# yhw-yhw/TalkSHOW

Hardware: NVIDIA H100
Metric: smplx_motion_frames_per_sec (higher is better)
Workload: dtype f32

## Files before the change

talkshow_b200/csrc/face.cu:

```cuda
#include <cuda_fp16.h>
#include "convstack.h"

#include <memory>
#include "pixelcnn.h"

namespace ts {

static const int W2V_K[7] = {10, 3, 3, 3, 3, 2, 2};
static const int W2V_S[7] = {5, 2, 2, 2, 2, 2, 2};

struct EncLayer {
  Layer qkv, out, ff1, ff2;
  float *ln1_g, *ln1_b, *ln2_g, *ln2_b;
};

struct FaceNet {
  float* conv0_w = nullptr;
  float *gn_g = nullptr, *gn_b = nullptr;
  Layer conv[7];
  float *fp_ln_g = nullptr, *fp_ln_b = nullptr;
  Layer fproj, posconv;
  unsigned short* pos_w16 = nullptr;
  float pos_unscale = 1.f;
  float *enc_ln_g = nullptr, *enc_ln_b = nullptr;
  std::vector<EncLayer> layers;
  Layer feat_map;
  float *id_w = nullptr, *id_b = nullptr;
  int ncls = 4;
  Layer fn_conv[3], fn_res0;
  float *fn_g[3], *fn_b[3];
  Layer dec_conv[2][3];
  float *dec_g[2][3], *dec_b[2][3];
  Layer fin[2];
  int jaw_dim = 3, exp_dim = 100;
};

void face_destroy(ts_engine* e) {
  delete e->face;
  e->face = nullptr;
}

static float* up(ts_engine* e, const float* p, size_t n) { return e->upload(std::vector<float>(p, p + n)); }

static Layer pack_ckc(ts_engine* e, const float* w, const float* b, int cout, int cin, int k) {
  int cp = pad4(cin);
  std::vector<float> W((size_t)cout * k * cp, 0.f);
  for (int o = 0; o < cout; ++o)
    for (int c = 0; c < cin; ++c)
      for (int t = 0; t < k; ++t) W[((size_t)o * k + t) * cp + c] = w[((size_t)o * cin + c) * k + t];
  Layer L;
  L.N = cout; L.taps = k; L.cin = cp; L.K = k * cp;
  upload_weights(e, W, &L);
  L.bias = b ? up(e, b, cout) : nullptr;
  return L;
}
static Layer pack_linear(ts_engine* e, const float* w, const float* b, int N, int K) {
  Layer L;
  L.N = N; L.K = K; L.taps = 1; L.cin = K;
  upload_weights(e, std::vector<float>(w, w + (size_t)N * K), &L);
  L.bias = b ? up(e, b, N) : nullptr;
  return L;
}

__global__ void __launch_bounds__(256) conv0_stats_kernel(const float* __restrict__ wave, const float* __restrict__ w, int N, int T0,
                                                          double* __restrict__ stats) {
  constexpr int TC = 256;
  __shared__ float xs[TC * 5 + 16];
  const int b = blockIdx.y, t0 = blockIdx.x * TC, tid = threadIdx.x;
  const int nt = min(TC, T0 - t0);
  const float* x = wave + (size_t)b * N + (size_t)t0 * 5;
  for (int i = tid; i < nt * 5 + 5; i += 256) xs[i] = x[i];
  __syncthreads();
  for (int c = tid; c < 512; c += 256) {
    float wr[10];
#pragma unroll
    for (int j = 0; j < 10; ++j) wr[j] = w[c * 10 + j];
    double s = 0.0, ss = 0.0;
    for (int t = 0; t < nt; ++t) {
      float y = 0.f;
#pragma unroll
      for (int j = 0; j < 10; ++j) y = fmaf(wr[j], xs[t * 5 + j], y);
      s += (double)y;
      ss += (double)y * (double)y;
    }
    atomicAdd(&stats[((size_t)b * 512 + c) * 2], s);
    atomicAdd(&stats[((size_t)b * 512 + c) * 2 + 1], ss);
  }
}
__global__ void __launch_bounds__(256) conv0_apply_kernel(const float* __restrict__ wave, const float* __restrict__ w,
                                                          const double* __restrict__ stats, const float* __restrict__ g,
                                                          const float* __restrict__ bta, int N, int T0, Act3 out) {
  constexpr int TC = 64;
  __shared__ float xs[TC * 5 + 16];
  const int b = blockIdx.y, t0 = blockIdx.x * TC, tid = threadIdx.x;
  const int nt = min(TC, T0 - t0);
  const float* x = wave + (size_t)b * N + (size_t)t0 * 5;
  for (int i = tid; i < nt * 5 + 5; i += 256) xs[i] = x[i];
  __syncthreads();
  for (int c = tid; c < 512; c += 256) {
    float wr[10];
#pragma unroll
    for (int j = 0; j < 10; ++j) wr[j] = w[c * 10 + j];
    double s = stats[((size_t)b * 512 + c) * 2], ss = stats[((size_t)b * 512 + c) * 2 + 1];
    double mean = s / T0, var = ss / T0 - mean * mean;
    if (var < 0) var = 0;
    float rstd = (float)(1.0 / sqrt(var + 1e-5)), mu = (float)mean, gg = g[c], bb = bta[c];
    for (int t = 0; t < nt; ++t) {
      float y = 0.f;
#pragma unroll
      for (int j = 0; j < 10; ++j) y = fmaf(wr[j], xs[t * 5 + j], y);
      float v = (y - mu) * rstd * gg + bb;
      v = 0.5f * v * (1.0f + erff(v * 0.70710678118654752440f));
      if (out.h16) {
        if (out.p) out.row(b, t0 + t)[c] = v;
        split16(v, out.row_h16(b, t0 + t)[c], out.row_l16(b, t0 + t)[c]);
      } else if (out.lo) {
        float h = __uint_as_float(__float_as_uint(v) & 0xffffe000u);
        out.row(b, t0 + t)[c] = h;
        out.row_lo(b, t0 + t)[c] = v - h;
      } else {
        out.row(b, t0 + t)[c] = v;
      }
    }
  }
}

__global__ void interp_kernel(Act3 in, Act3 out) {
  const float scale = (float)in.T / (float)out.T;
  long n = (long)out.B * out.T * out.C;
  for (long i = blockIdx.x * (long)blockDim.x + threadIdx.x; i < n; i += (long)gridDim.x * blockDim.x) {
    int c = i % out.C;
    long bt = i / out.C;
    int t = bt % out.T, b = bt / out.T;
    float src = __fsub_rn(__fmul_rn(scale, (float)t + 0.5f), 0.5f);
    if (src < 0.f) src = 0.f;
    int i0 = (int)src;
    if (i0 > in.T - 1) i0 = in.T - 1;
    int i1 = i0 + (i0 < in.T - 1 ? 1 : 0);
    float l1 = src - (float)i0, l0 = 1.0f - l1;
    out.row(b, t)[c] = l0 * in.row(b, i0)[c] + l1 * in.row(b, i1)[c];
  }
}

__global__ void ln_pre_kernel(Act3 x, Act3 pre, int has_pre, const float* __restrict__ g, const float* __restrict__ bta, Act3 y,
                              Act3 res, int has_res, int act, float eps) {
  int warp = (blockIdx.x * blockDim.x + threadIdx.x) >> 5, lane = threadIdx.x & 31;
  int rows = x.B * x.T;
  if (warp >= rows) return;
  int b = warp / x.T, t = warp % x.T, C = x.C;
  const float* xr = x.row(b, t);
  const float* xl = x.lo ? x.row_lo(b, t) : nullptr;
  const float* pr = has_pre ? pre.row(b, t) : nullptr;
  float v[24];
  float s = 0.f;
  int n = 0;
  for (int c = lane; c < C; c += 32, ++n) {
    float a = xr[c];
    if (xl) a += xl[c];
    if (pr) a += pr[c];
    v[n] = a;
    s += a;
  }
  for (int o = 16; o > 0; o >>= 1) s += __shfl_xor_sync(0xffffffffu, s, o);
  float mean = s / C, q = 0.f;
  for (int i = 0; i < n; ++i) { float d = v[i] - mean; q = fmaf(d, d, q); }
  for (int o = 16; o > 0; o >>= 1) q += __shfl_xor_sync(0xffffffffu, q, o);
  float rstd = 1.0f / sqrtf(q / C + eps);
  float* yr = y.row(b, t);
  float* yl = y.lo ? y.row_lo(b, t) : nullptr;
  const float* rr = has_res ? res.row(b, t) : nullptr;
  const float* rl = (has_res && res.lo) ? res.row_lo(b, t) : nullptr;
  n = 0;
  for (int c = lane; c < C; c += 32, ++n) {
    float o = (v[n] - mean) * rstd * g[c] + bta[c];
    if (rr) o += rl ? (rr[c] + rl[c]) : rr[c];
    if (act == ACT_RELU) o = o > 0.f ? o : 0.f;
    if (y.h16) {
      yr[c] = o;
      split16(o, y.row_h16(b, t)[c], y.row_l16(b, t)[c]);
    } else if (yl) {
      float h = __uint_as_float(__float_as_uint(o) & 0xffffe000u);
      yr[c] = h;
      yl[c] = o - h;
    } else {
      yr[c] = o;
    }
  }
}
static void ln_pre(ts_engine* e, const Act3& x, const Act3* pre, const float* g, const float* b, const Act3& y, const Act3* res,
                   int act, cudaStream_t s) {
  if (e->ws.sizing) return;
  if (x.C > 768) fail(TS_ERR_INVALID, "layernorm width %d > 768", x.C);
  int rows = x.B * x.T;
  ln_pre_kernel<<<cdiv(rows, 8), 256, 0, s>>>(x, pre ? *pre : Act3(), pre ? 1 : 0, g, b, y, res ? *res : Act3(), res ? 1 : 0, act, 1e-5f);
  e->launches++;
  TS_CUDA(cudaGetLastError());
}

__global__ void id_cols_kernel(const float* __restrict__ idv, const float* __restrict__ w, const float* __restrict__ bias, int ncls,
                               Act3 x, int off) {
  int b = blockIdx.y;
  __shared__ float v[64];
  if (threadIdx.x < 64) {
    float a = bias[threadIdx.x];
    for (int k = 0; k < ncls; ++k) a = fmaf(w[threadIdx.x * ncls + k], idv[b * ncls + k], a);
// ... 929 lines not shown
      e->launches++;
      TS_CUDA(cudaGetLastError());
      return;
    }
  }
  const int Tp = (T + 63) & ~63;
  auto smem = [&](int QT) { return (size_t)(QT * 65 + 64 * 65 + QT * Tp) * sizeof(float); };
  const float scale = 0.125f;
  const size_t lim = 220 * 1024;
  if (smem(64) <= lim) {
    TS_CUDA(cudaFuncSetAttribute(attention_kernel<64>, cudaFuncAttributeMaxDynamicSharedMemorySize, (int)smem(64)));
    attention_kernel<64><<<dim3(cdiv(T, 64), B * H), 256, smem(64), s>>>(qkv, out, out_lo, T, H, scale);
  } else if (smem(32) <= lim) {
    TS_CUDA(cudaFuncSetAttribute(attention_kernel<32>, cudaFuncAttributeMaxDynamicSharedMemorySize, (int)smem(32)));
    attention_kernel<32><<<dim3(cdiv(T, 32), B * H), 256, smem(32), s>>>(qkv, out, out_lo, T, H, scale);
  } else if (smem(16) <= lim) {
    TS_CUDA(cudaFuncSetAttribute(attention_kernel<16>, cudaFuncAttributeMaxDynamicSharedMemorySize, (int)smem(16)));
    attention_kernel<16><<<dim3(cdiv(T, 16), B * H), 256, smem(16), s>>>(qkv, out, out_lo, T, H, scale);
  } else {
    fail(TS_ERR_UNSUPPORTED, "attention: %d frames exceed the shared-memory score tile (max ~3000 frames = 100 s)", T);
  }
  e->launches++;
  TS_CUDA(cudaGetLastError());
}

static void linear(ts_engine* e, const Layer& L, const Act3& x, const Act3& y, int act, const Act3* res, cudaStream_t s, int coff = 0) {
  if (L.K != x.C) fail(TS_ERR_INVALID, "linear: K %d vs C %d", L.K, x.C);
  conv_auto(e, L, x, 1, 1, 0, y, x.T, act, res, s, 1, 0, coff);
}

static void face_run(ts_engine* e, const float* wave, const float* idv, float* out, int B, int N, int frame, cudaStream_t s) {
  FaceNet& F = *e->face;
  int T = (N - 10) / 5 + 1;
  double* stats = e->ws.alloc<double>((size_t)B * 512 * 2);
  const bool tc = e->use_tc;
  Act3 h = new_act(e, B, T, 512, 0, s, tc, T & 1, true);
  if (!e->ws.sizing) {
    TS_CUDA(cudaMemsetAsync(stats, 0, (size_t)B * 512 * 2 * sizeof(double), s));
    conv0_stats_kernel<<<dim3(cdiv(T, 256), B), 256, 0, s>>>(wave, F.conv0_w, N, T, stats);
    conv0_apply_kernel<<<dim3(cdiv(T, 64), B), 256, 0, s>>>(wave, F.conv0_w, stats, F.gn_g, F.gn_b, N, T, h);
    e->launches += 2;
    TS_CUDA(cudaGetLastError());
  }
  for (int i = 1; i < 7; ++i) {
    int To = (T - W2V_K[i]) / W2V_S[i] + 1;
    Act3 y = new_act(e, B, To, 512, 0, s, tc && i < 6, To & 1, true);
    conv_auto(e, F.conv[i], h, W2V_K[i], W2V_S[i], 0, y, To, ACT_GELU, nullptr, s);
    h = y;
    T = To;
  }
  Act3 hi = new_act(e, B, frame, 512, 0, s);
  if (!e->ws.sizing) {
    long n = (long)B * frame * 512;
    interp_kernel<<<(int)std::min<long>((n + 255) / 256, (long)e->sm_count * 16), 256, 0, s>>>(h, hi);
    e->launches++;
    TS_CUDA(cudaGetLastError());
  }
  Act3 hn = new_act(e, B, frame, 512, 0, s, tc);
  ln_pre(e, hi, nullptr, F.fp_ln_g, F.fp_ln_b, hn, nullptr, ACT_NONE, s);
  Act3 x = new_act(e, B, frame, 768, 64, s);
  linear(e, F.fproj, hn, x, ACT_NONE, nullptr, s);
  Act3 pc = new_act(e, B, frame, 768, 0, s);
  if (e->use_tc && F.pos_w16) {
    if (!e->ws.sizing) {
      TS_CUDA(cudaFuncSetAttribute(posconv_mma_kernel, cudaFuncAttributeMaxDynamicSharedMemorySize, (int)PC_SMEM));
      posconv_mma_kernel<<<dim3(B * 16, cdiv(frame, PC_ROWS)), PC_WARPS * 32, PC_SMEM, s>>>(x, F.pos_w16, F.posconv.bias, F.pos_unscale, pc);
      e->launches++;
      TS_CUDA(cudaGetLastError());
    }
  } else {
    GemmP p;
    p.A = x.row(0, -64); p.W = F.posconv.W; p.bias = F.posconv.bias; p.C = pc.row(0, 0);
    p.M = B * frame; p.N = 48; p.K = 128 * 48; p.mper = frame;
    p.a_bs = x.bstride(); p.a_rs = 768; p.kc = 48; p.a_ts = 768;
    p.c_bs = pc.bstride(); p.c_rs = 768; p.act = ACT_GELU; p.ldw = 128 * 48;
    p.groups = 16; p.a_goff = 48; p.w_goff = (long)48 * 128 * 48; p.n_goff = 48;
    launch_gemm(e, p, s);
  }
  Act3 hcur = new_act(e, B, frame, 768, 0, s, tc);
  ln_pre(e, x, &pc, F.enc_ln_g, F.enc_ln_b, hcur, nullptr, ACT_NONE, s);
  Act3 qkv = new_act(e, B, frame, 2304, 0, s);
  Act3 att = new_act(e, B, frame, 768, 0, s, tc);
  Act3 t1 = new_act(e, B, frame, 768, 0, s);
  Act3 ff = new_act(e, B, frame, 3072, 0, s, tc);
  for (auto& L : F.layers) {
    linear(e, L.qkv, hcur, qkv, ACT_NONE, nullptr, s);
    attention(e, qkv.p, att, B, frame, 12, s);
    linear(e, L.out, att, t1, ACT_NONE, &hcur, s);
    ln_pre(e, t1, nullptr, L.ln1_g, L.ln1_b, hcur, nullptr, ACT_NONE, s);
    linear(e, L.ff1, hcur, ff, ACT_GELU, nullptr, s);
    linear(e, L.ff2, ff, t1, ACT_NONE, &hcur, s);
    ln_pre(e, t1, nullptr, L.ln2_g, L.ln2_b, hcur, nullptr, ACT_NONE, s);
  }
  const bool tcf = tc && e->tc_f16;
  Act3 cat = new_act(e, B, frame, 320, 1, s, tcf);
  linear(e, F.feat_map, hcur, cat, ACT_NONE, nullptr, s, 0);
  if (!e->ws.sizing) {
    id_cols_kernel<<<dim3(cdiv(frame * 64, 256), B), 256, 0, s>>>(idv, F.id_w, F.id_b, F.ncls, cat, 256);
    e->launches++;
    TS_CUDA(cudaGetLastError());
  }
  Act3 c0 = new_act(e, B, frame, 256, 0, s), r0 = new_act(e, B, frame, 256, 0, s);
  conv_auto(e, F.fn_conv[0], cat, 3, 1, 1, c0, frame, ACT_NONE, nullptr, s);
  conv_auto(e, F.fn_res0, cat, 3, 1, 1, r0, frame, ACT_NONE, nullptr, s);
  Act3 f = new_act(e, B, frame, 256, 1, s, tcf);
  ln_pre(e, c0, nullptr, F.fn_g[0], F.fn_b[0], f, &r0, ACT_RELU, s);
  for (int i = 1; i < 3; ++i) {
    conv_auto(e, F.fn_conv[i], f, 3, 1, 1, c0, frame, ACT_NONE, nullptr, s);
    Act3 g = new_act(e, B, frame, 256, 1, s, tcf);
    ln_pre(e, c0, nullptr, F.fn_g[i], F.fn_b[i], g, &f, ACT_RELU, s);
    f = g;
  }
  Act3 yout;
  yout.p = out; yout.B = B; yout.T = frame; yout.C = F.jaw_dim + F.exp_dim; yout.pad = 0;
  for (int br = 0; br < 2; ++br) {
    int c = br ? 256 : 64;
    Act3 m = f;
    for (int i = 0; i < 3; ++i) {
      Act3 cc = new_act(e, B, frame, c, 0, s);
      conv_auto(e, F.dec_conv[br][i], m, 3, 1, 1, cc, frame, ACT_NONE, nullptr, s);
      Act3 nn = new_act(e, B, frame, c, 1, s, tcf);
      ln_pre(e, cc, nullptr, F.dec_g[br][i], F.dec_b[br][i], nn, nullptr, ACT_RELU, s);
      m = nn;
    }
    linear(e, F.fin[br], m, yout, ACT_NONE, nullptr, s, br ? F.jaw_dim : 0);
  }
}

}

using namespace ts;

extern "C" int ts_load_face(ts_engine* e, const ts_tensor* tensors, int n) {
  TS_API_BEGIN(e)
  Ckpt ck(tensors, n);
  LoadScope scope(e, "face");
  std::unique_ptr<FaceNet> Fp(new FaceNet());
  FaceNet* F = Fp.get();
  const std::string a = "audio_encoder.";
  F->conv0_w = up(e, ck.f32(a + "feature_extractor.conv_layers.0.conv.weight", {512, 1, 10}), 5120);
  F->gn_g = up(e, ck.f32(a + "feature_extractor.conv_layers.0.layer_norm.weight", {512}), 512);
  F->gn_b = up(e, ck.f32(a + "feature_extractor.conv_layers.0.layer_norm.bias", {512}), 512);
  for (int i = 1; i < 7; ++i)
    F->conv[i] = pack_ckc(e, ck.f32(a + "feature_extractor.conv_layers." + std::to_string(i) + ".conv.weight", {512, 512, W2V_K[i]}),
                          nullptr, 512, 512, W2V_K[i]);
  F->fp_ln_g = up(e, ck.f32(a + "feature_projection.layer_norm.weight", {512}), 512);
  F->fp_ln_b = up(e, ck.f32(a + "feature_projection.layer_norm.bias", {512}), 512);
  F->fproj = pack_linear(e, ck.f32(a + "feature_projection.projection.weight", {768, 512}),
                         ck.f32(a + "feature_projection.projection.bias", {768}), 768, 512);
  const std::string en = a + "encoder.";
  F->posconv = pack_ckc(e, ck.f32(en + "pos_conv_embed.conv.weight", {768, 48, 128}), ck.f32(en + "pos_conv_embed.conv.bias", {768}),
                        768, 48, 128);
  F->pos_w16 = pack_posconv16(e, ck.f32(en + "pos_conv_embed.conv.weight", {768, 48, 128}), &F->pos_unscale);
  F->enc_ln_g = up(e, ck.f32(en + "layer_norm.weight", {768}), 768);
  F->enc_ln_b = up(e, ck.f32(en + "layer_norm.bias", {768}), 768);
  for (int l = 0; ck.has(en + "layers." + std::to_string(l) + ".attention.q_proj.weight"); ++l) {
    const std::string p = en + "layers." + std::to_string(l) + ".";
    EncLayer L;
    std::vector<float> W((size_t)2304 * 768), Bv(2304);
    const char* nm[3] = {"q_proj", "k_proj", "v_proj"};
    for (int j = 0; j < 3; ++j) {
      const float* w = ck.f32(p + "attention." + nm[j] + ".weight", {768, 768});
      const float* b = ck.f32(p + "attention." + nm[j] + ".bias", {768});
      std::copy(w, w + (size_t)768 * 768, W.begin() + (size_t)j * 768 * 768);
      std::copy(b, b + 768, Bv.begin() + j * 768);
    }
    L.qkv.N = 2304; L.qkv.K = 768; L.qkv.taps = 1; L.qkv.cin = 768;
// ... 66 lines not shown
```

talkshow_b200/csrc/gemm_tc.cu:

```cuda
#include <cuda.h>
#include <cuda_fp16.h>

#include "kernels.h"

namespace ts {

constexpr int TC_BM = 128, TC_BN = 128;
constexpr int TC_BK = 32;
constexpr int TC_STAGES = 3;
constexpr int TC_TILE_BYTES = 128 * 128;
constexpr int TC_STAGE_BYTES = 4 * TC_TILE_BYTES;
constexpr int TC_THREADS = 384;
constexpr int TC_SMEM = TC_STAGES * TC_STAGE_BYTES + 1024  + 256 ;
constexpr int TC_SLD = TC_BN + 4;
static_assert(TC_BM * TC_SLD * 4 + 2 * TC_BM * 8 <= TC_STAGES * TC_STAGE_BYTES, "parked tile must fit in the operand ring");
static_assert(TC_SMEM <= 227 * 1024, "shared memory per block");

struct TcArgs {
  int taps, cblocks, stride;
  int C;
  int rows_in, off, T_out, nbatch;
  int Rs;
  int N;
  float* c_hi;
  float* c_lo;
  long c_bs, c_rs;
  const float* bias;
  const float* r_hi;
  const float* r_lo;
  long r_bs, r_rs;
  int act;
  int chunk;
  float oscale;
  unsigned short* c_h16;
  unsigned short* c_l16;
};

__device__ __forceinline__ uint32_t s_u32(const void* p) { return (uint32_t)__cvta_generic_to_shared(p); }
__device__ __forceinline__ void mb_init(uint64_t* b, int c) { asm volatile("mbarrier.init.shared::cta.b64 [%0], %1;" ::"r"(s_u32(b)), "r"(c)); }
__device__ __forceinline__ void mb_expect(uint64_t* b, uint32_t bytes) {
  asm volatile("mbarrier.arrive.expect_tx.shared::cta.b64 _, [%0], %1;" ::"r"(s_u32(b)), "r"(bytes) : "memory");
}
__device__ __forceinline__ void mb_arrive_lane0(uint64_t* b, int lane) {
  asm volatile("{\n.reg .pred p;\nsetp.eq.s32 p, %1, 0;\n@p mbarrier.arrive.shared::cta.b64 _, [%0];\n}\n" ::"r"(s_u32(b)), "r"(lane) : "memory");
}
__device__ __forceinline__ void mb_wait(uint64_t* b, uint32_t parity) {
  asm volatile(
      "{\n.reg .pred p;\nTCW:\nmbarrier.try_wait.parity.shared::cta.b64 p, [%0], %1;\n@p bra TCD;\nbra TCW;\nTCD:\n}\n" ::"r"(s_u32(b)),
      "r"(parity)
      : "memory");
}
__device__ __forceinline__ void tma_3d(void* dst, const CUtensorMap* m, int c0, int c1, int c2, uint64_t* bar) {
  asm volatile("cp.async.bulk.tensor.3d.shared::cluster.global.tile.mbarrier::complete_tx::bytes [%0], [%1, {%2, %3, %4}], [%5];" ::"r"(s_u32(dst)),
               "l"(m), "r"(c0), "r"(c1), "r"(c2), "r"(s_u32(bar))
               : "memory");
}
__device__ __forceinline__ void tma_2d(void* dst, const CUtensorMap* m, int c0, int c1, uint64_t* bar) {
  asm volatile("cp.async.bulk.tensor.2d.shared::cluster.global.tile.mbarrier::complete_tx::bytes [%0], [%1, {%2, %3}], [%4];" ::"r"(s_u32(dst)),
               "l"(m), "r"(c0), "r"(c1), "r"(s_u32(bar))
               : "memory");
}
__device__ __forceinline__ uint64_t wg_desc(uint32_t smem_addr) {
  uint64_t d = 0;
  d |= (uint64_t)((smem_addr >> 4) & 0x3fff);
  d |= (uint64_t)1 << 16;
  d |= (uint64_t)(1024 >> 4) << 32;
  d |= (uint64_t)1 << 62;
  return d;
}
#define TC_ACC64                                                                                                              \
  "{%0, %1, %2, %3, %4, %5, %6, %7, %8, %9, %10, %11, %12, %13, %14, %15, %16, %17, %18, %19, %20, %21, %22, %23, %24, %25, " \
  "%26, %27, %28, %29, %30, %31, %32, %33, %34, %35, %36, %37, %38, %39, %40, %41, %42, %43, %44, %45, %46, %47, %48, %49, "   \
  "%50, %51, %52, %53, %54, %55, %56, %57, %58, %59, %60, %61, %62, %63}"
#define TC_ACC64_OPS(d)                                                                                                       \
  "+f"(d[0]), "+f"(d[1]), "+f"(d[2]), "+f"(d[3]), "+f"(d[4]), "+f"(d[5]), "+f"(d[6]), "+f"(d[7]), "+f"(d[8]), "+f"(d[9]),     \
      "+f"(d[10]), "+f"(d[11]), "+f"(d[12]), "+f"(d[13]), "+f"(d[14]), "+f"(d[15]), "+f"(d[16]), "+f"(d[17]), "+f"(d[18]),    \
      "+f"(d[19]), "+f"(d[20]), "+f"(d[21]), "+f"(d[22]), "+f"(d[23]), "+f"(d[24]), "+f"(d[25]), "+f"(d[26]), "+f"(d[27]),    \
      "+f"(d[28]), "+f"(d[29]), "+f"(d[30]), "+f"(d[31]), "+f"(d[32]), "+f"(d[33]), "+f"(d[34]), "+f"(d[35]), "+f"(d[36]),    \
      "+f"(d[37]), "+f"(d[38]), "+f"(d[39]), "+f"(d[40]), "+f"(d[41]), "+f"(d[42]), "+f"(d[43]), "+f"(d[44]), "+f"(d[45]),    \
      "+f"(d[46]), "+f"(d[47]), "+f"(d[48]), "+f"(d[49]), "+f"(d[50]), "+f"(d[51]), "+f"(d[52]), "+f"(d[53]), "+f"(d[54]),    \
      "+f"(d[55]), "+f"(d[56]), "+f"(d[57]), "+f"(d[58]), "+f"(d[59]), "+f"(d[60]), "+f"(d[61]), "+f"(d[62]), "+f"(d[63])
template <bool F16>
__device__ __forceinline__ void wgmma_64x128(float (&d)[64], uint64_t a, uint64_t b, int scale_d) {
  if constexpr (F16)
    asm volatile("{\n.reg .pred p;\nsetp.ne.b32 p, %66, 0;\n"
                 "wgmma.mma_async.sync.aligned.m64n128k16.f32.f16.f16 " TC_ACC64 ", %64, %65, p, 1, 1, 0, 0;\n}\n"
                 : TC_ACC64_OPS(d)
                 : "l"(a), "l"(b), "r"(scale_d));
  else
    asm volatile("{\n.reg .pred p;\nsetp.ne.b32 p, %66, 0;\n"
                 "wgmma.mma_async.sync.aligned.m64n128k8.f32.tf32.tf32 " TC_ACC64 ", %64, %65, p, 1, 1;\n}\n"
                 : TC_ACC64_OPS(d)
                 : "l"(a), "l"(b), "r"(scale_d));
}
#undef TC_ACC64
#undef TC_ACC64_OPS
__device__ __forceinline__ void wgmma_fence() { asm volatile("wgmma.fence.sync.aligned;" ::: "memory"); }
__device__ __forceinline__ void wgmma_commit() { asm volatile("wgmma.commit_group.sync.aligned;" ::: "memory"); }
template <int N>
__device__ __forceinline__ void wgmma_wait() { asm volatile("wgmma.wait_group.sync.aligned %0;" ::"n"(N) : "memory"); }

__device__ __forceinline__ float tc_act(float v, int act) {
  if (act == ACT_RELU) return v > 0.f ? v : 0.f;
  if (act == ACT_LRELU) return v > 0.f ? v : 0.2f * v;
  if (act == ACT_GELU) return 0.5f * v * (1.0f + erff(v * 0.70710678118654752440f));
  return v;
}

template <int ACT, int CG, int SLD>
__device__ __forceinline__ void tc_writeout(const TcArgs& P, const float* S, const long* rowc, const long* rowr, int n0) {
  const int et = threadIdx.x - 128;
  const int c4 = (et % CG) * 4, n = n0 + c4;
  if (n >= P.N) return;
  const int nv = min(4, P.N - n);
  float bv[4] = {0.f, 0.f, 0.f, 0.f};
  if (P.bias)
    for (int q = 0; q < nv; ++q) bv[q] = P.bias[n + q];
  const float osc = P.oscale;
  const bool rvec = nv == 4 && P.r_hi && (((P.r_bs | P.r_rs) & 3) == 0) && ((reinterpret_cast<uintptr_t>(P.r_hi) & 15) == 0) &&
                    (!P.r_lo || (reinterpret_cast<uintptr_t>(P.r_lo) & 15) == 0);
#pragma unroll 4
  for (int r = et / CG; r < TC_BM; r += 256 / CG) {
    const long co = rowc[r];
    if (co < 0) continue;
    const float4 sv = *reinterpret_cast<const float4*>(&S[r * SLD + c4]);
    float o[4] = {sv.x * osc + bv[0], sv.y * osc + bv[1], sv.z * osc + bv[2], sv.w * osc + bv[3]};
    if (P.r_hi) {
      const long roff = rowr[r] + n;
      if (rvec) {
        const float4 rh = *reinterpret_cast<const float4*>(P.r_hi + roff);
        if (P.r_lo) {
          const float4 rl = *reinterpret_cast<const float4*>(P.r_lo + roff);
          o[0] += rh.x + rl.x; o[1] += rh.y + rl.y; o[2] += rh.z + rl.z; o[3] += rh.w + rl.w;
        } else {
          o[0] += rh.x; o[1] += rh.y; o[2] += rh.z; o[3] += rh.w;
        }
      } else {
        for (int q = 0; q < nv; ++q) o[q] += P.r_lo ? (P.r_hi[roff + q] + P.r_lo[roff + q]) : P.r_hi[roff + q];
      }
    }
#pragma unroll
    for (int q = 0; q < 4; ++q) {
      if (ACT == ACT_GELU) o[q] = 0.5f * o[q] * (1.0f + erff(o[q] * 0.70710678118654752440f));
      else if (ACT != ACT_NONE) o[q] = tc_act(o[q], P.act);
    }
    const long coff = co + n;
    if (nv == 4) {
      if (P.c_h16) {
        if (P.c_hi) *reinterpret_cast<float4*>(P.c_hi + coff) = make_float4(o[0], o[1], o[2], o[3]);
        ushort4 h, l;
        split16(o[0], h.x, l.x); split16(o[1], h.y, l.y); split16(o[2], h.z, l.z); split16(o[3], h.w, l.w);
        *reinterpret_cast<ushort4*>(P.c_h16 + coff) = h;
        *reinterpret_cast<ushort4*>(P.c_l16 + coff) = l;
      } else if (P.c_lo) {
        float4 h, l;
        h.x = __uint_as_float(__float_as_uint(o[0]) & 0xffffe000u); l.x = o[0] - h.x;
        h.y = __uint_as_float(__float_as_uint(o[1]) & 0xffffe000u); l.y = o[1] - h.y;
        h.z = __uint_as_float(__float_as_uint(o[2]) & 0xffffe000u); l.z = o[2] - h.z;
        h.w = __uint_as_float(__float_as_uint(o[3]) & 0xffffe000u); l.w = o[3] - h.w;
        *reinterpret_cast<float4*>(P.c_hi + coff) = h;
        *reinterpret_cast<float4*>(P.c_lo + coff) = l;
      } else {
        *reinterpret_cast<float4*>(P.c_hi + coff) = make_float4(o[0], o[1], o[2], o[3]);
      }
    } else {
      for (int q = 0; q < nv; ++q) {
        if (P.c_h16) {
          if (P.c_hi) P.c_hi[coff + q] = o[q];
          split16(o[q], P.c_h16[coff + q], P.c_l16[coff + q]);
        } else if (P.c_lo) {
          const float h = __uint_as_float(__float_as_uint(o[q]) & 0xffffe000u);
          P.c_hi[coff + q] = h;
          P.c_lo[coff + q] = o[q] - h;
        } else {
          P.c_hi[coff + q] = o[q];
        }
      }
    }
  }
}

template <bool F16>
__global__ void __launch_bounds__(TC_THREADS, 1)
tc_gemm_kernel(const __grid_constant__ CUtensorMap mA_hi, const __grid_constant__ CUtensorMap mA_lo,
               const __grid_constant__ CUtensorMap mB_hi, const __grid_constant__ CUtensorMap mB_lo, TcArgs P) {
  extern __shared__ unsigned char tc_smem_raw[];
  unsigned char* smem = reinterpret_cast<unsigned char*>((reinterpret_cast<uintptr_t>(tc_smem_raw) + 1023) & ~uintptr_t(1023));
  uint64_t* full = reinterpret_cast<uint64_t*>(smem + TC_STAGES * TC_STAGE_BYTES);
  uint64_t* empty = full + TC_STAGES;
  const int warp = threadIdx.x >> 5, lane = threadIdx.x & 31;
  const int j0 = blockIdx.y * TC_BM, n0 = blockIdx.x * TC_BN;
  const int nk = P.taps * P.cblocks;
  constexpr int BK = F16 ? 2 * TC_BK : TC_BK;

  if (threadIdx.x == 0) {
    for (int i = 0; i < TC_STAGES; ++i) { mb_init(&full[i], 1); mb_init(&empty[i], 8); }
    asm volatile("fence.mbarrier_init.release.cluster;" ::: "memory");
    asm volatile("prefetch.tensormap [%0];" ::"l"(&mA_hi) : "memory");
    asm volatile("prefetch.tensormap [%0];" ::"l"(&mA_lo) : "memory");
    asm volatile("prefetch.tensormap [%0];" ::"l"(&mB_hi) : "memory");
    asm volatile("prefetch.tensormap [%0];" ::"l"(&mB_lo) : "memory");
  }
  __syncthreads();

  if (warp < 4) {
    if (threadIdx.x == 0) {
      for (int kb = 0; kb < nk; ++kb) {
        const int st = kb % TC_STAGES, ph = (kb / TC_STAGES) & 1;
        mb_wait(&empty[st], ph ^ 1);
        const int tap = kb / P.cblocks, cb = kb - tap * P.cblocks;
        unsigned char* base = smem + st * TC_STAGE_BYTES;
        mb_expect(&full[st], TC_STAGE_BYTES);
        const int c0 = cb * BK, c1 = tap % P.stride, c2 = j0 + tap / P.stride;
        const int kcol = tap * P.C + cb * BK;
        tma_3d(base, &mA_hi, c0, c1, c2, &full[st]);
        tma_3d(base + TC_TILE_BYTES, &mA_lo, c0, c1, c2, &full[st]);
        tma_2d(base + 2 * TC_TILE_BYTES, &mB_hi, kcol, n0, &full[st]);
        tma_2d(base + 3 * TC_TILE_BYTES, &mB_lo, kcol, n0, &full[st]);
      }
    }
    return;
  }

  const int wg = (warp >> 2) - 1;
  float acc[64], sum[64];
#pragma unroll
  for (int i = 0; i < 64; ++i) sum[i] = 0.f;
  for (int c0 = 0; c0 < nk; c0 += P.chunk) {
    const int cend = min(nk, c0 + P.chunk);
    for (int kb = c0; kb < cend; ++kb) {
      const int st = kb % TC_STAGES, ph = (kb / TC_STAGES) & 1;
      mb_wait(&full[st], ph);
      const uint32_t a_hi = s_u32(smem + st * TC_STAGE_BYTES) + wg * 64 * 128, a_lo = a_hi + TC_TILE_BYTES;
      const uint32_t b_hi = s_u32(smem + st * TC_STAGE_BYTES) + 2 * TC_TILE_BYTES, b_lo = b_hi + TC_TILE_BYTES;
      wgmma_fence();
#pragma unroll
      for (int k = 0; k < 4; ++k) {
        const uint32_t o = k * 32;
        wgmma_64x128<F16>(acc, wg_desc(a_lo + o), wg_desc(b_hi + o), (kb > c0) | k);
        wgmma_64x128<F16>(acc, wg_desc(a_hi + o), wg_desc(b_lo + o), 1);
        wgmma_64x128<F16>(acc, wg_desc(a_hi + o), wg_desc(b_hi + o), 1);
      }
      wgmma_commit();
      wgmma_wait<1>();
      __syncwarp();
      if (kb > c0) mb_arrive_lane0(&empty[(kb + TC_STAGES - 1) % TC_STAGES], lane);
    }
    wgmma_wait<0>();
    __syncwarp();
    mb_arrive_lane0(&empty[(cend - 1) % TC_STAGES], lane);
#pragma unroll
    for (int i = 0; i < 64; ++i) sum[i] += acc[i];
  }

  asm volatile("bar.sync 1, 256;" ::: "memory");
  float* S = reinterpret_cast<float*>(smem);
  long* rowc = reinterpret_cast<long*>(S + TC_BM * TC_SLD);
  long* rowr = rowc + TC_BM;
  {
    const int r0 = wg * 64 + (warp & 3) * 16 + (lane >> 2), c0 = 2 * (lane & 3);
#pragma unroll
    for (int i = 0; i < 64; i += 2) {
      const int r = r0 + 8 * ((i >> 1) & 1), c = c0 + 8 * (i >> 2);
      *reinterpret_cast<float2*>(&S[r * TC_SLD + c]) = make_float2(sum[i], sum[i + 1]);
    }
  }
  const int et = threadIdx.x - 128;
  if (et < TC_BM) {
    const int j = j0 + et;
    long co = -1, ro = 0;
    if (j < P.Rs) {
      const long in_row = (long)j * P.stride;
      const int bb = (int)(in_row / P.rows_in);
      const int tin = (int)(in_row - (long)bb * P.rows_in) - P.off;
      if (bb < P.nbatch && tin >= 0 && (tin % P.stride) == 0 && tin / P.stride < P.T_out) {
        const int t = tin / P.stride;
        co = (long)bb * P.c_bs + (long)t * P.c_rs;
        ro = (long)bb * P.r_bs + (long)t * P.r_rs;
      }
    }
    rowc[et] = co;
    rowr[et] = ro;
  }
  asm volatile("bar.sync 1, 256;" ::: "memory");
  if (P.act == ACT_NONE) tc_writeout<ACT_NONE, TC_BN / 4, TC_SLD>(P, S, rowc, rowr, n0);
  else if (P.act == ACT_GELU) tc_writeout<ACT_GELU, TC_BN / 4, TC_SLD>(P, S, rowc, rowr, n0);
  else tc_writeout<-1, TC_BN / 4, TC_SLD>(P, S, rowc, rowr, n0);
}

__global__ void split_kernel(const float* __restrict__ x, float* __restrict__ hi, float* __restrict__ lo, long n) {
  for (long i = blockIdx.x * (long)blockDim.x + threadIdx.x; i < n; i += (long)gridDim.x * blockDim.x) {
    float v = x[i];
    float h = __uint_as_float(__float_as_uint(v) & 0xffffe000u);
    hi[i] = h;
    lo[i] = v - h;
  }
}
void split_hi_lo(ts_engine* e, const float* x, float* hi, float* lo, long n, cudaStream_t s) {
  if (e->ws.sizing || n <= 0) return;
  split_kernel<<<(int)std::min<long>((n + 255) / 256, (long)e->sm_count * 16), 256, 0, s>>>(x, hi, lo, n);
  e->launches++;
  TS_CUDA(cudaGetLastError());
}
__global__ void split16_kernel(const float* __restrict__ x, unsigned short* __restrict__ h, unsigned short* __restrict__ l, long n, float scale) {
  for (long i = blockIdx.x * (long)blockDim.x + threadIdx.x; i < n; i += (long)gridDim.x * blockDim.x) split16(x[i] * scale, h[i], l[i]);
}
static float split16_host(const std::vector<float>& w, std::vector<unsigned short>* h, std::vector<unsigned short>* l) {
  float mx = 0.f;
  for (float v : w) mx = std::max(mx, std::fabs(v));
  int shift = 0;
  if (mx > 0.f && std::isfinite(mx)) {
    int ex;
    std::frexp(mx, &ex);
    shift = std::min(14, std::max(0, 14 - ex));
  }
  const float sc = std::ldexp(1.0f, shift);
  h->resize(w.size());
  l->resize(w.size());
  for (size_t i = 0; i < w.size(); ++i) {
    const float v = w[i] * sc;
    const __half hh = __float2half_rn(v);
    const __half ll = __float2half_rn(v - __half2float(hh));
    (*h)[i] = __half_as_ushort(hh);
    (*l)[i] = __half_as_ushort(ll);
  }
  return std::ldexp(1.0f, -shift);
}
void split_host(const std::vector<float>& w, std::vector<float>* hi, std::vector<float>* lo) {
  hi->resize(w.size());
  lo->resize(w.size());
  for (size_t i = 0; i < w.size(); ++i) {
    uint32_t u;
    memcpy(&u, &w[i], 4);
    u &= 0xffffe000u;
    float h;
    memcpy(&h, &u, 4);
    (*hi)[i] = h;
    (*lo)[i] = w[i] - h;
  }
}

typedef CUresult (*EncodeTiledFn)(CUtensorMap*, CUtensorMapDataType, cuuint32_t, void*, const cuuint64_t*, const cuuint64_t*,
                                  const cuuint32_t*, const cuuint32_t*, CUtensorMapInterleave, CUtensorMapSwizzle,
                                  CUtensorMapL2promotion, CUtensorMapFloatOOBfill);
static EncodeTiledFn get_encode() {
  static EncodeTiledFn fn = nullptr;
  if (!fn) {
    void* p = nullptr;
    cudaDriverEntryPointQueryResult q;
    TS_CUDA(cudaGetDriverEntryPoint("cuTensorMapEncodeTiled", &p, cudaEnableDefault, &q));
    if (!p || q != cudaDriverEntryPointSuccess) fail(TS_ERR_CUDA, "cuTensorMapEncodeTiled entry point unavailable");
    fn = (EncodeTiledFn)p;
  }
  return fn;
}
static CUtensorMap make_map(const void* base, int rank, const cuuint64_t* dims, const cuuint64_t* strides_bytes, const cuuint32_t* box,
                            bool f16 = false) {
  CUtensorMap m;
  cuuint32_t estr[3] = {1, 1, 1};
  CUresult r = get_encode()(&m, f16 ? CU_TENSOR_MAP_DATA_TYPE_FLOAT16 : CU_TENSOR_MAP_DATA_TYPE_FLOAT32, rank, (void*)base, dims, strides_bytes, box, estr, CU_TENSOR_MAP_INTERLEAVE_NONE,
                            CU_TENSOR_MAP_SWIZZLE_128B, CU_TENSOR_MAP_L2_PROMOTION_L2_256B, CU_TENSOR_MAP_FLOAT_OOB_FILL_NONE);
  if (r != CUDA_SUCCESS) fail(TS_ERR_CUDA, "cuTensorMapEncodeTiled failed (%d) rank %d dims %llu,%llu", (int)r, rank, (unsigned long long)dims[0],
                              (unsigned long long)dims[1]);
  return m;
}

bool tc_conv_supported(ts_engine* e, const Layer& L, const Act3& x, int stride, int pd) {
// ... 144 lines not shown
```

Baseline: 193,800.

## Vectorize conv0 stores, precompute GEMM row map in producer warps, widen epilogue

The conv0 apply kernel now handles two adjacent channels per thread and writes paired float2/ushort2 stores instead of scalar ones. In the tensor-core GEMM, the producer warpgroup's idle warps compute the output row-offset tables into a dedicated shared region while the MMA runs. The epilogue writeout then uses all 384 threads after a full __syncthreads instead of only the 256 consumer threads. The ff activation buffer also gets an extra allocation flag, which may change its precision or layout, so these are several unrelated changes touching memory traffic and epilogue parallelism.

```diff
diff --git a/talkshow_b200/csrc/face.cu b/talkshow_b200/csrc/face.cu
--- a/talkshow_b200/csrc/face.cu
+++ b/talkshow_b200/csrc/face.cu
@@ -97,30 +97,46 @@
   const float* x = wave + (size_t)b * N + (size_t)t0 * 5;
   for (int i = tid; i < nt * 5 + 5; i += 256) xs[i] = x[i];
   __syncthreads();
-  for (int c = tid; c < 512; c += 256) {
-    float wr[10];
-#pragma unroll
-    for (int j = 0; j < 10; ++j) wr[j] = w[c * 10 + j];
-    double s = stats[((size_t)b * 512 + c) * 2], ss = stats[((size_t)b * 512 + c) * 2 + 1];
-    double mean = s / T0, var = ss / T0 - mean * mean;
+  const int c = 2 * tid;
+  float wr[2][10], rstd[2], mu[2], gg[2], bb[2];
+#pragma unroll
+  for (int q = 0; q < 2; ++q) {
+#pragma unroll
+    for (int j = 0; j < 10; ++j) wr[q][j] = w[(c + q) * 10 + j];
+    const double s = stats[((size_t)b * 512 + c + q) * 2], ss = stats[((size_t)b * 512 + c + q) * 2 + 1];
+    const double mean = s / T0;
+    double var = ss / T0 - mean * mean;
     if (var < 0) var = 0;
-    float rstd = (float)(1.0 / sqrt(var + 1e-5)), mu = (float)mean, gg = g[c], bb = bta[c];
-    for (int t = 0; t < nt; ++t) {
+    rstd[q] = (float)(1.0 / sqrt(var + 1e-5));
+    mu[q] = (float)mean;
+    gg[q] = g[c + q];
+    bb[q] = bta[c + q];
+  }
+  for (int t = 0; t < nt; ++t) {
+    float v[2];
+#pragma unroll
+    for (int q = 0; q < 2; ++q) {
       float y = 0.f;
 #pragma unroll
-      for (int j = 0; j < 10; ++j) y = fmaf(wr[j], xs[t * 5 + j], y);
-      float v = (y - mu) * rstd * gg + bb;
-      v = 0.5f * v * (1.0f + erff(v * 0.70710678118654752440f));
-      if (out.h16) {
-        if (out.p) out.row(b, t0 + t)[c] = v;
-        split16(v, out.row_h16(b, t0 + t)[c], out.row_l16(b, t0 + t)[c]);
-      } else if (out.lo) {
-        float h = __uint_as_float(__float_as_uint(v) & 0xffffe000u);
-        out.row(b, t0 + t)[c] = h;
-        out.row_lo(b, t0 + t)[c] = v - h;
-      } else {
-        out.row(b, t0 + t)[c] = v;
-      }
+      for (int j = 0; j < 10; ++j) y = fmaf(wr[q][j], xs[t * 5 + j], y);
+      v[q] = (y - mu[q]) * rstd[q] * gg[q] + bb[q];
+      v[q] = 0.5f * v[q] * (1.0f + erff(v[q] * 0.70710678118654752440f));
+    }
+    if (out.h16) {
+      if (out.p) *reinterpret_cast<float2*>(out.row(b, t0 + t) + c) = make_float2(v[0], v[1]);
+      ushort2 h, l;
+      split16(v[0], h.x, l.x);
+      split16(v[1], h.y, l.y);
+      *reinterpret_cast<ushort2*>(out.row_h16(b, t0 + t) + c) = h;
+      *reinterpret_cast<ushort2*>(out.row_l16(b, t0 + t) + c) = l;
+    } else if (out.lo) {
+      float2 h, l;
+      h.x = __uint_as_float(__float_as_uint(v[0]) & 0xffffe000u); l.x = v[0] - h.x;
+      h.y = __uint_as_float(__float_as_uint(v[1]) & 0xffffe000u); l.y = v[1] - h.y;
+      *reinterpret_cast<float2*>(out.row(b, t0 + t) + c) = h;
+      *reinterpret_cast<float2*>(out.row_lo(b, t0 + t) + c) = l;
+    } else {
+      *reinterpret_cast<float2*>(out.row(b, t0 + t) + c) = make_float2(v[0], v[1]);
     }
   }
 }
@@ -1216,7 +1232,7 @@
   Act3 qkv = new_act(e, B, frame, 2304, 0, s);
   Act3 att = new_act(e, B, frame, 768, 0, s, tc);
   Act3 t1 = new_act(e, B, frame, 768, 0, s);
-  Act3 ff = new_act(e, B, frame, 3072, 0, s, tc);
+  Act3 ff = new_act(e, B, frame, 3072, 0, s, tc, 0, true);
   for (auto& L : F.layers) {
     linear(e, L.qkv, hcur, qkv, ACT_NONE, nullptr, s);
     attention(e, qkv.p, att, B, frame, 12, s);
diff --git a/talkshow_b200/csrc/gemm_tc.cu b/talkshow_b200/csrc/gemm_tc.cu
--- a/talkshow_b200/csrc/gemm_tc.cu
+++ b/talkshow_b200/csrc/gemm_tc.cu
@@ -11,9 +11,9 @@
 constexpr int TC_TILE_BYTES = 128 * 128;
 constexpr int TC_STAGE_BYTES = 4 * TC_TILE_BYTES;
 constexpr int TC_THREADS = 384;
-constexpr int TC_SMEM = TC_STAGES * TC_STAGE_BYTES + 1024  + 256 ;
+constexpr int TC_SMEM = TC_STAGES * TC_STAGE_BYTES + 1024  + 2 * TC_BM * 8  + 256 ;
 constexpr int TC_SLD = TC_BN + 4;
-static_assert(TC_BM * TC_SLD * 4 + 2 * TC_BM * 8 <= TC_STAGES * TC_STAGE_BYTES, "parked tile must fit in the operand ring");
+static_assert(TC_BM * TC_SLD * 4 <= TC_STAGES * TC_STAGE_BYTES, "parked tile must fit in the operand ring");
 static_assert(TC_SMEM <= 227 * 1024, "shared memory per block");
 
 struct TcArgs {
@@ -109,7 +109,7 @@
 
 template <int ACT, int CG, int SLD>
 __device__ __forceinline__ void tc_writeout(const TcArgs& P, const float* S, const long* rowc, const long* rowr, int n0) {
-  const int et = threadIdx.x - 128;
+  const int et = threadIdx.x;
   const int c4 = (et % CG) * 4, n = n0 + c4;
   if (n >= P.N) return;
   const int nv = min(4, P.N - n);
@@ -120,7 +120,7 @@
   const bool rvec = nv == 4 && P.r_hi && (((P.r_bs | P.r_rs) & 3) == 0) && ((reinterpret_cast<uintptr_t>(P.r_hi) & 15) == 0) &&
                     (!P.r_lo || (reinterpret_cast<uintptr_t>(P.r_lo) & 15) == 0);
 #pragma unroll 4
-  for (int r = et / CG; r < TC_BM; r += 256 / CG) {
+  for (int r = et / CG; r < TC_BM; r += TC_THREADS / CG) {
     const long co = rowc[r];
     if (co < 0) continue;
     const float4 sv = *reinterpret_cast<const float4*>(&S[r * SLD + c4]);
@@ -186,7 +186,9 @@
                const __grid_constant__ CUtensorMap mB_hi, const __grid_constant__ CUtensorMap mB_lo, TcArgs P) {
   extern __shared__ unsigned char tc_smem_raw[];
   unsigned char* smem = reinterpret_cast<unsigned char*>((reinterpret_cast<uintptr_t>(tc_smem_raw) + 1023) & ~uintptr_t(1023));
-  uint64_t* full = reinterpret_cast<uint64_t*>(smem + TC_STAGES * TC_STAGE_BYTES);
+  long* rowc = reinterpret_cast<long*>(smem + TC_STAGES * TC_STAGE_BYTES);
+  long* rowr = rowc + TC_BM;
+  uint64_t* full = reinterpret_cast<uint64_t*>(rowr + TC_BM);
   uint64_t* empty = full + TC_STAGES;
   const int warp = threadIdx.x >> 5, lane = threadIdx.x & 31;
   const int j0 = blockIdx.y * TC_BM, n0 = blockIdx.x * TC_BN;
@@ -218,46 +220,58 @@
         tma_2d(base + 2 * TC_TILE_BYTES, &mB_hi, kcol, n0, &full[st]);
         tma_2d(base + 3 * TC_TILE_BYTES, &mB_lo, kcol, n0, &full[st]);
       }
+    } else if (warp > 0) {
+      for (int r = threadIdx.x - 32; r < TC_BM; r += 96) {
+        const int j = j0 + r;
+        long co = -1, ro = 0;
+        if (j < P.Rs) {
+          const long in_row = (long)j * P.stride;
+          const int bb = (int)(in_row / P.rows_in);
+          const int tin = (int)(in_row - (long)bb * P.rows_in) - P.off;
+          if (bb < P.nbatch && tin >= 0 && (tin % P.stride) == 0 && tin / P.stride < P.T_out) {
+            const int t = tin / P.stride;
+            co = (long)bb * P.c_bs + (long)t * P.c_rs;
+            ro = (long)bb * P.r_bs + (long)t * P.r_rs;
+          }
+        }
+        rowc[r] = co;
+        rowr[r] = ro;
+      }
     }
-    return;
-  }
-
-  const int wg = (warp >> 2) - 1;
-  float acc[64], sum[64];
+  } else {
+    const int wg = (warp >> 2) - 1;
+    float acc[64], sum[64];
 #pragma unroll
-  for (int i = 0; i < 64; ++i) sum[i] = 0.f;
-  for (int c0 = 0; c0 < nk; c0 += P.chunk) {
-    const int cend = min(nk, c0 + P.chunk);
-    for (int kb = c0; kb < cend; ++kb) {
-      const int st = kb % TC_STAGES, ph = (kb / TC_STAGES) & 1;
-      mb_wait(&full[st], ph);
-      const uint32_t a_hi = s_u32(smem + st * TC_STAGE_BYTES) + wg * 64 * 128, a_lo = a_hi + TC_TILE_BYTES;
-      const uint32_t b_hi = s_u32(smem + st * TC_STAGE_BYTES) + 2 * TC_TILE_BYTES, b_lo = b_hi + TC_TILE_BYTES;
-      wgmma_fence();
+    for (int i = 0; i < 64; ++i) sum[i] = 0.f;
+    for (int c0 = 0; c0 < nk; c0 += P.chunk) {
+      const int cend = min(nk, c0 + P.chunk);
+      for (int kb = c0; kb < cend; ++kb) {
+        const int st = kb % TC_STAGES, ph = (kb / TC_STAGES) & 1;
+        mb_wait(&full[st], ph);
+        const uint32_t a_hi = s_u32(smem + st * TC_STAGE_BYTES) + wg * 64 * 128, a_lo = a_hi + TC_TILE_BYTES;
+        const uint32_t b_hi = s_u32(smem + st * TC_STAGE_BYTES) + 2 * TC_TILE_BYTES, b_lo = b_hi + TC_TILE_BYTES;
+        wgmma_fence();
 #pragma unroll
-      for (int k = 0; k < 4; ++k) {
-        const uint32_t o = k * 32;
-        wgmma_64x128<F16>(acc, wg_desc(a_lo + o), wg_desc(b_hi + o), (kb > c0) | k);
-        wgmma_64x128<F16>(acc, wg_desc(a_hi + o), wg_desc(b_lo + o), 1);
-        wgmma_64x128<F16>(acc, wg_desc(a_hi + o), wg_desc(b_hi + o), 1);
+        for (int k = 0; k < 4; ++k) {
+          const uint32_t o = k * 32;
+          wgmma_64x128<F16>(acc, wg_desc(a_lo + o), wg_desc(b_hi + o), (kb > c0) | k);
+          wgmma_64x128<F16>(acc, wg_desc(a_hi + o), wg_desc(b_lo + o), 1);
+          wgmma_64x128<F16>(acc, wg_desc(a_hi + o), wg_desc(b_hi + o), 1);
+        }
+        wgmma_commit();
+        wgmma_wait<1>();
+        __syncwarp();
+        if (kb > c0) mb_arrive_lane0(&empty[(kb + TC_STAGES - 1) % TC_STAGES], lane);
       }
-      wgmma_commit();
-      wgmma_wait<1>();
+      wgmma_wait<0>();
       __syncwarp();
-      if (kb > c0) mb_arrive_lane0(&empty[(kb + TC_STAGES - 1) % TC_STAGES], lane);
+      mb_arrive_lane0(&empty[(cend - 1) % TC_STAGES], lane);
+#pragma unroll
+      for (int i = 0; i < 64; ++i) sum[i] += acc[i];
     }
-    wgmma_wait<0>();
-    __syncwarp();
-    mb_arrive_lane0(&empty[(cend - 1) % TC_STAGES], lane);
-#pragma unroll
-    for (int i = 0; i < 64; ++i) sum[i] += acc[i];
-  }
-
-  asm volatile("bar.sync 1, 256;" ::: "memory");
-  float* S = reinterpret_cast<float*>(smem);
-  long* rowc = reinterpret_cast<long*>(S + TC_BM * TC_SLD);
-  long* rowr = rowc + TC_BM;
-  {
+
+    asm volatile("bar.sync 1, 256;" ::: "memory");
+    float* S = reinterpret_cast<float*>(smem);
     const int r0 = wg * 64 + (warp & 3) * 16 + (lane >> 2), c0 = 2 * (lane & 3);
 #pragma unroll
     for (int i = 0; i < 64; i += 2) {
@@ -265,24 +279,8 @@
       *reinterpret_cast<float2*>(&S[r * TC_SLD + c]) = make_float2(sum[i], sum[i + 1]);
     }
   }
-  const int et = threadIdx.x - 128;
-  if (et < TC_BM) {
-    const int j = j0 + et;
-    long co = -1, ro = 0;
-    if (j < P.Rs) {
-      const long in_row = (long)j * P.stride;
-      const int bb = (int)(in_row / P.rows_in);
-      const int tin = (int)(in_row - (long)bb * P.rows_in) - P.off;
-      if (bb < P.nbatch && tin >= 0 && (tin % P.stride) == 0 && tin / P.stride < P.T_out) {
-        const int t = tin / P.stride;
-        co = (long)bb * P.c_bs + (long)t * P.c_rs;
-        ro = (long)bb * P.r_bs + (long)t * P.r_rs;
-      }
-    }
-    rowc[et] = co;
-    rowr[et] = ro;
-  }
-  asm volatile("bar.sync 1, 256;" ::: "memory");
+  __syncthreads();
+  const float* S = reinterpret_cast<const float*>(smem);
   if (P.act == ACT_NONE) tc_writeout<ACT_NONE, TC_BN / 4, TC_SLD>(P, S, rowc, rowr, n0);
   else if (P.act == ACT_GELU) tc_writeout<ACT_GELU, TC_BN / 4, TC_SLD>(P, S, rowc, rowr, n0);
   else tc_writeout<-1, TC_BN / 4, TC_SLD>(P, S, rowc, rowr, n0);
```

New measurement: 199,200 (median of 6 runs). +2.8%, better.
